# genomicepidemiology/ccphylo

Hardware: AMD Instinct MI355X
Metric: taxa-pairs/sec (dist) + NJ iterations/sec at N taxa, 1/2/4/8 MI355X (higher is better)
Workload: dtype u2 packed codes -> MX-fp4 MFMA (exact integer counts), f64 LT and tree

## Files before the change

### ccphylo_amd/csrc/ccg_dnj_form.h

```cpp
#pragma once
#include <stdlib.h>

#ifdef __HIPCC__
#define CCG_FORM_HD __host__ __device__ __forceinline__
#else
#define CCG_FORM_HD inline
#endif

#define DNJ_B 128
#define DNJ_BANDS 64
#define DNJ_BANDS_MAX 128
#define SEG 2048
#define TBF 1024
#define FIND_RPT 16
#define PLAN_MAXB 256
#define UHIST 64

CCG_FORM_HD int dnj_umax(int n, int seg) { return n > 2 ? (n - 2) / seg + 1 : 1; }

struct DnjGrid {
	int scan_div = 4, scan_max = 2048, seg_mul = 0, prefold_n = 0;
	int small_wave = 0, adapt_rows = 500;
	int sphase_b = 512;
	int plan_help = 256;
	int scan_cmp = 1, cmp_blocks = 1024;
	long long prune_cells = 20000000;
	int prune_on = 1;
	int s_top = 0, s_bands = -1, s_split_n = 16384, plan_qdelay = 2, scan_wave = -1, plan_multi = 1;
	int plan_regsel = 0, plan_fr = FIND_RPT;
	int test_withhold = 0;
	int join_pf = 1;
	int scan_fold = 0;
	int scan_prune = 2;
	int lb = 1, lb_min_n = 16384;
	int lb_groups = 0;
	int scan_vblk = 1;
	void load() {
		if(const char *e = getenv("CCG_JOIN_PF")) join_pf = atoi(e);
		if(const char *e = getenv("CCG_SCAN_FOLD")) scan_fold = atoi(e);
		if(const char *e = getenv("CCG_SCAN_PRUNE")) scan_prune = atoi(e);
		if(const char *e = getenv("CCG_SCAN_VBLK")) scan_vblk = atoi(e);
		if(const char *e = getenv("CCG_S_TOP")) s_top = atoi(e) > 0 ? atoi(e) : 0;
		if(const char *e = getenv("CCG_S_BANDS")) s_bands = atoi(e) >= 0 ? atoi(e) : -1;
		if(const char *e = getenv("CCG_S_SPLIT_N")) s_split_n = atoi(e);
		if(const char *e = getenv("CCG_SCAN_DIV")) scan_div = atoi(e) > 0 ? atoi(e) : 4;
		if(const char *e = getenv("CCG_SCAN_MAX")) scan_max = atoi(e) > 0 ? atoi(e) : 2048;
		if(const char *e = getenv("CCG_SEG_MUL")) seg_mul = atoi(e) > 0 ? atoi(e) : 0;
		if(const char *e = getenv("CCG_PREFOLD_N")) prefold_n = atoi(e) >= 0 ? atoi(e) : 0;
		if(const char *e = getenv("CCG_SCAN_ADAPT")) adapt_rows = atoi(e) > 0 ? atoi(e) : 0;
		if(const char *e = getenv("CCG_SPHASE_BLOCKS")) sphase_b = atoi(e) > 0 ? atoi(e) : 512;
		if(const char *e = getenv("CCG_PLAN_HELP")) plan_help = atoi(e) >= 0 && atoi(e) < 512 ? atoi(e) : 256;
		if(const char *e = getenv("CCG_SCAN_CMP")) scan_cmp = atoi(e);
		if(const char *e = getenv("CCG_PRUNE_CELLS")) prune_cells = atoll(e) > 0 ? atoll(e) : 0;
		prune_on = 1;
		if(const char *e = getenv("CCG_SCAN_CMPB")) cmp_blocks = atoi(e) > 0 ? atoi(e) : 1024;
		if(const char *e = getenv("CCG_PLAN_QDELAY")) plan_qdelay = atoi(e) >= 0 ? atoi(e) : 2;
		if(const char *e = getenv("CCG_SCAN_WAVE")) scan_wave = atoi(e);
		if(const char *e = getenv("CCG_PLAN_MULTI")) plan_multi = atoi(e);
		if(const char *e = getenv("CCG_PLAN_REGSEL")) plan_regsel = atoi(e);
		if(const char *e = getenv("CCG_PLAN_FR")) plan_fr = atoi(e) < 1 ? 1 : atoi(e) > FIND_RPT ? FIND_RPT : atoi(e);
		if(const char *e = getenv("CCG_TEST_WITHHOLD")) test_withhold = atoi(e) & 3;
		if(const char *e = getenv("CCG_SCAN_LB")) lb = atoi(e);
		if(const char *e = getenv("CCG_LB_MIN_N")) lb_min_n = atoi(e);
		if(const char *e = getenv("CCG_LB_GROUPS")) lb_groups = atoi(e);
	}
	int plan_flags(bool prune = false, int helpers = 0) const {
		return (plan_qdelay & 0x3fff) | (test_withhold & 3) << 14 | (plan_regsel ? 0 : 1 << 16) | ((plan_fr - 1) & 15) << 17 | (prune ? 1 << 21 : 0) |
		       (helpers & 511) << 22;
	}
	unsigned plan_blocks(int n) const {
		if(!plan_multi) return 1;
		const int step = (TBF - 64) * plan_fr;
		const int g = (n - 1 + step - 1) / step;
		return (unsigned) (g < 1 ? 1 : g > PLAN_MAXB ? PLAN_MAXB : g);
	}
	int scan_mode(int n, int et = 8) const {
		return scan_wave >= 0 ? scan_wave : n > 16384 || small_wave ? (et == 8 ? 9 : 20) : 0;
	}
	int seg(int n) const {
		int m = seg_mul ? seg_mul : n / (8 * SEG);
		m = m < 1 ? 1 : m > 8 ? 8 : m;
		return m * SEG;
	}
	bool prefold(int n) const { return n > prefold_n; }
	int top(int n) const {
		const int t = s_top ? s_top : n > s_split_n ? 16 : DNJ_B;
		return t < 1 ? 1 : t > DNJ_B ? DNJ_B : t;
	}
	int bands(int n) const {
		int b = s_bands >= 0 ? s_bands : n > s_split_n ? DNJ_BANDS : 0;
		b = b > DNJ_BANDS_MAX ? DNJ_BANDS_MAX : b;
		return top(n) + b > DNJ_B ? DNJ_B - top(n) : b;
	}
	unsigned sphase_blocks() const { return sphase_b; }
	unsigned scan(int n) const {
		const long long g = (n + scan_div - 1) / scan_div;
		return (unsigned) (g < scan_max ? g : scan_max);
	}
};

enum ScanKernel {
	SCAN_BLOCK,
	SCAN_WAVE,
	SCAN_WAVE16,
	SCAN_GROUP,
	SCAN_GROUP_CMP
};
enum ScanSphase {
	SPHASE_NONE,
	SPHASE_SCAN,
	SPHASE_COMPACT
};
struct ScanForm {
	ScanKernel kernel;
	bool stream;
	int G, UC;
	int prune;
	bool cmp;
	bool lb;
	bool tfold;
	int helpers;
	ScanSphase sphase;
	bool fold;
	int sfold;
	unsigned grid;
	int launches;
};

inline int dnj_scan_base(int sm) {
	return sm <= 0 ? 0 : sm < 4 ? 1 : sm == 9 || sm == 21 || sm > 23 ? sm : sm < 20 ? 4 : 20;
}

inline ScanForm dnj_scan_form(const DnjGrid &g, int n, int et, bool gen, bool have_lbm) {
	const int sm = dnj_scan_base(g.scan_mode(n, et));
	const bool grp = sm == 20 || sm == 21, prefold = g.prefold(n);
	const bool fits = dnj_umax(n, g.seg(n)) < UHIST;
	ScanForm f = {};
	f.tfold = prefold && g.scan_fold && sm >= 1;
	if(!gen && g.bands(n) && prefold && sm >= 4 && sm <= 23) {
		if(g.scan_prune == 1 && g.scan_fold) f.prune = 1;
		else if(g.scan_prune == 2 && g.prune_on && !g.scan_fold && (!grp || (g.scan_cmp && fits))) f.prune = 2;
	}
	f.helpers = f.prune == 2 ? g.plan_help : 0;
	f.sphase = f.prune != 2 ? SPHASE_NONE : g.plan_help ? SPHASE_COMPACT : SPHASE_SCAN;
	f.cmp = !gen && sm >= 4 && g.scan_cmp && !f.tfold && f.prune != 1 && fits;
	if(gen || sm < 4) f.kernel = sm >= 1 ? SCAN_WAVE : SCAN_BLOCK;
	else if(have_lbm && f.cmp && grp && g.lb_groups && f.prune == 0) {
		f.kernel = SCAN_GROUP_CMP;
		f.lb = true;
		f.G = 4;
		f.UC = 8;
	} else if(have_lbm && f.cmp) {
		f.kernel = SCAN_WAVE16;
		f.lb = true;
	} else if(grp) {
		f.kernel = f.cmp ? SCAN_GROUP_CMP : SCAN_GROUP;
		f.G = sm == 21 ? 8 : 4;
		f.UC = sm == 21 ? 4 : 8;
	} else {
		f.kernel = SCAN_WAVE16;
		f.stream = sm == 9;
	}
	f.grid = f.cmp && g.scan(n) > (unsigned) g.cmp_blocks ? (unsigned) g.cmp_blocks : g.scan(n);
	f.fold = prefold && !f.tfold;
	f.sfold = f.prune == 2;
	f.launches = 1 + (f.sphase != SPHASE_NONE) + f.fold;
	return f;
// ... 13 lines not shown
```

### ccphylo_amd/csrc/ccg_dnj_search.h

```cpp
#pragma once
#include <stdlib.h>
#include "ccg_tree_common.h"
#include "ccg_dnj_form.h"

struct DenseRows {
	__host__ __device__ __forceinline__ bool owns(long long) const { return true; }
	__host__ __device__ __forceinline__ long long row(long long r) const { return tri(r); }
};

#define SEG_S 1024
#define SEL_RPL 8
#define SEL_STEPS 8
#define FIND_CHUNKS 2048
#define REPLAY_CAP 2048
#define JOIN_UPRE 2048
#define FOLD_BLOCKS 256
#define SRDY_REP 64


template <int ET, bool GEN, int NT, int UNR, class Rows>
__device__ __forceinline__ void row_segment_min(const Rows &rows, const typename Elem<ET>::T *__restrict__ D, double bs,
                                                const double *__restrict__ sD, const int *__restrict__ N, int r,
                                                int c0, int c1, int Nr, double sDr, int isub, int Nm, double sDm,
                                                double &q, int &idx) {
// ... 696 lines not shown
	}
	TSW(1, 10, 64);
	__syncthreads();
	TS(1, 1);
	if(s_done) return;
	auto count_prefix = [&]() {
		constexpr int NC = FR * LW, PER = (NC + 63) / 64;
		int c[PER], sum = 0;
#pragma unroll
		for(int k = 0; k < PER; ++k) {
			const int x = lane * PER + k;
			c[k] = x < NC ? s_mw[x] : 0;
			sum += c[k];
		}
		int tot;
		int pre = wave_excl_scan(sum, &tot);
#pragma unroll
		for(int k = 0; k < PER; ++k) {
			const int x = lane * PER + k;
			if(x < NC) s_mw[x] = pre;
			pre += c[k];
		}
		if(lane == 0) s_cnt = tot;
		return tot;
	};
	if(regsel) {
		const int jsub = s_jsub, isub = s_isub;
		const double m0 = s_m0;
		unsigned long long bs_[FR];
#pragma unroll
		for(int m = 0; m < FR; ++m) {
			bs_[m] = 0ull;
			if(wid > 0) {
				const int r = top - (m * LT + lt);
				qv[m] = r == jsub ? s_Qj : r == isub ? s_Qi : qv[m];
				bs_[m] = __ballot(r >= 1 && qv[m] < m0);
				if(lane == 0) s_mw[m * LW + wid - 1] = __popcll(bs_[m]);
			}
		}
		__syncthreads();
		if(wid == 0) count_prefix();
		__syncthreads();
		const int tot = s_cnt, nt = tot < ktop ? tot : ktop;
		long long ctop = 0;
#pragma unroll
		for(int m = 0; m < FR; ++m) {
			if(bs_[m] == 0ull) continue;
			const int r = top - (m * LT + lt);
			const int pos = s_mw[m * LW + wid - 1] + (int) __builtin_amdgcn_mbcnt_hi(
			                    (unsigned) (bs_[m] >> 32), __builtin_amdgcn_mbcnt_lo((unsigned) bs_[m], 0));
			if(((bs_[m] >> lane) & 1ull) && pos < ktop) {
				sS[pos] = r;
				sQS[pos] = qv[m];
				b.crow[pos] = r;
				b.cbnd[pos] = qv[m];
				if(bid == 0) atomicAdd(&s_uh[dcdiv(r, seg) < UHIST ? dcdiv(r, seg) : UHIST - 1], 1);
				ctop += rows.owns(r) ? r : 0;
			}
		}
		ctop = wave_sum_int(ctop);
		if(lane == 0 && ctop) {
			atomicAdd((unsigned long long *) &ctl->cells, (unsigned long long) ctop);
			atomicAdd((unsigned long long *) &ctl->cells_top, (unsigned long long) ctop);
		}
		__syncthreads();
		if(tid == 0) {
			const int sm = nt == ktop ? sS[ktop - 1] : 1;
			s_nS = s_ntop = nt;
			s_smin = sm;
			ctl->smin = sm;
		}
		__syncthreads();
	}
	const int nS = s_nS, ntop = s_ntop, smin = s_smin, isub = s_isub, jsub = s_jsub;
	const double m0 = s_m0;
	if(wid > 0) {
		double qp = DBL_MAX;
		if(have_rt && rt != isub && rt != jsub && 0 <= dpr) {
			const bool pm = pr == isub;
			qp = qcrit(GEN ? nr : n, GEN ? (pm ? s_Nm : np) : n, dpr, sdr, pm ? s_sDm : sdp);
		}
		spq[lt] = qp;
	}
	TSW(1, 11, 64);
	__syncthreads();
	double U;
	{
		double v = DBL_MAX;
		if(tid < nS) {
			const int r = sS[tid];
			const double qk = tid >= ntop ? sQP[tid] : top - r < NSP ? spq[top - r] : DBL_MAX;
			const double Qk = sQS[tid];
			v = qk > Qk ? qk : Qk;
		}
		const double x = wave_incl_min(v);
		if(wid < 2 && lane == 63) spm[DNJ_B + wid] = x;
		__syncthreads();
		double c = m0;
		if(wid == 1) c = spm[DNJ_B] < c ? spm[DNJ_B] : c;
		if(tid < nS) spm[tid] = x < c ? x : c;
		__syncthreads();
		U = ntop ? spm[ntop - 1] : m0;
	}
	TS(1, 2);
	const bool bands = BANDS && nS > ntop;
	const int nch0 = smin > 1 && bands ? ((smin - 1) >> 6) + 1 : 0;
	const bool table = nch0 <= FIND_CHUNKS;
	const int nch = table ? nch0 : 0;
	for(int c = tid; c < nch; c += TBF) {
		int lo = ntop, hi = nS;
		while(lo < hi) {
			const int mid = (lo + hi) >> 1;
			if(sS[mid] >= 64 * (c + 1)) lo = mid + 1; else hi = mid;
		}
		sch[c] = lo;
	}
	if(nch) __syncthreads();
	auto s_above = [&](int r) {
		int k;
		if(table) {
			k = sch[r >> 6];
			while(k < nS && sS[k] > r) ++k;
		} else {
			int lo = ntop, hi = nS;
			while(lo < hi) {
				const int mid = (lo + hi) >> 1;
				if(sS[mid] > r) lo = mid + 1; else hi = mid;
			}
			k = lo;
		}
		return k;
	};
	int T = ntop, listed = 0;
	long long mycells = 0;
	if(smin > 1 && top - bstep >= 1) {
		double qn[FR];
		for(int base = top - bstep; base >= 1; base -= stride) {
			if(base != top - bstep && wid > 0) {
#pragma unroll
				for(int m = 0; m < FR; ++m) qv[m] = qn[m];
			}
			if(bands) {
				if(tid < FR * LW) {
					const int w = tid / FR, m = tid - (tid / FR) * FR;
					const int rh0 = base - (m * LT + w * 64), rhi = rh0 < smin - 1 ? rh0 : smin - 1;
					const int t0 = rhi >= 1 ? s_above(rhi) : nS;
					s_sb[tid] = t0 ? spm[t0 - 1] : m0;
					s_sf[tid] = t0 < nS && sS[t0] >= rh0 - 63;
				}
				__syncthreads();
			}
			unsigned sfm = 0;
			if(bands && wid > 0) {
				const uint4 f4 = *(const uint4 *) (s_sf + (wid - 1) * FR);
				const unsigned fw[4] = {f4.x, f4.y, f4.z, f4.w};
#pragma unroll
				for(int m = 0; m < FR; ++m) sfm |= ((fw[m >> 2] >> (8 * (m & 3))) & 1u) << m;
			}
			if(base == top) TS(1, 5);
			unsigned long long bm[FR];
			unsigned sbm = 0;
#pragma unroll
			for(int m = 0; m < FR; ++m) bm[m] = 0ull;
			const int mlim = (base - 1) / LT + 1 < fr ? (base - 1) / LT + 1 : fr;
#pragma unroll
			for(int m = 0; m < FR; ++m) {
				if(m >= mlim) continue;
				const int r = wid > 0 ? base - (m * LT + lt) : 0;
				const int rhi = base - (m * LT + (wid - 1) * 64);
				if((jsub <= rhi && jsub >= rhi - 63) || (isub <= rhi && isub >= rhi - 63))
					qv[m] = r == jsub ? s_Qj : r == isub ? s_Qi : qv[m];
				double bnd = U;
				bool srow = false;
				if(bands && wid > 0) {
					if((sfm >> m) & 1u) {
						const int t = s_above(r);
						srow = t < nS && sS[t] == r;
						bnd = t ? spm[t - 1] : m0;
					} else {
						bnd = s_sb[(wid - 1) * FR + m];
					}
				}
				bool f = false;
				if(r >= 1 && r < smin && rows.owns(r)) f = srow || qv[m] < bnd;
				sbm |= (f && srow ? 1u : 0u) << m;
				bm[m] = __ballot(f);
				if(lane == 0 && wid > 0) s_mw[m * LW + wid - 1] = __popcll(bm[m]);
			}
			if(lane == 0 && wid > 0) {
#pragma unroll
				for(int m = 0; m < FR; ++m)
					if(m >= mlim) s_mw[m * LW + wid - 1] = 0;
			}
			if(wid > 0 && base - stride >= 1) {
#pragma unroll
				for(int m = 0; m < FR; ++m) {
					const int r = base - stride - (m * LT + lt);
					qn[m] = m < fr && r >= 1 ? b.Q[r] : DBL_MAX;
				}
			}
			TSW(1, 12, 64);
			if(base == top) TSW(1, 6, 64);
			__syncthreads();
			if(wid == 0) {
				const int tot = count_prefix();
				if(nblk > 1) {
					if(lane == 0 && !(wh_cnt && bid == 0))
						__hip_atomic_store(b.ppub + bid, ((unsigned long long) n << 32) | (unsigned) tot,
						                   __ATOMIC_RELAXED, __HIP_MEMORY_SCOPE_AGENT);
					int off = 0;
					bool stuck = false;
					for(int g0 = 0; g0 < bid; g0 += 64) {
						const int g = g0 + lane;
						unsigned long long u = 0;
						bool ok = g >= bid;
						for(int spin = 0;; ++spin) {
							if(!ok) {
								u = __hip_atomic_load(b.ppub + g, __ATOMIC_RELAXED, __HIP_MEMORY_SCOPE_AGENT);
								ok = (int) (u >> 32) == n;
							}
							if(__all(ok)) break;
							if(spin > spin_max) {
								stuck = true;
								break;
							}
							__builtin_amdgcn_s_sleep(1);
						}
						off += wave_sum_int(g < bid && ok ? (int) (u & 0xffffffffu) : 0);
					}
					if(lane == 0) {
						s_off = off;
						if(stuck) {
							ctl->final_n = -1;
							ctl->done = 1;
						}
					}
				}
				TS(1, 13);
				if(base == top) TS(1, 7);
			}
			__syncthreads();
			if(nblk > 1 && base == top - bstep) T += s_off;
#pragma unroll
			for(int m = 0; m < FR; ++m) {
				if(bm[m] == 0ull) continue;
				const int r = base - (m * LT + lt);
				const bool f = (bm[m] >> lane) & 1ull;
				mycells += f ? r : 0;
				{
					const int rh = base - (m * LT + (wid - 1) * 64), bh0 = dcdiv(rh, seg);
					const int bh = bh0 < UHIST ? bh0 : UHIST - 1;
					const int ch = __popcll(__ballot(f && dcdiv(r, seg) == bh0)), ct = __popcll(bm[m]);
					if(lane == 0) {
						atomicAdd(&s_uh[bh], ch);
						if(ct > ch) atomicAdd(&s_uh[bh0 - 1 < UHIST ? bh0 - 1 : UHIST - 1], ct - ch);
					}
				}
				if(f) {
					const int pos = T + s_mw[m * LW + wid - 1] +
					                (int) __builtin_amdgcn_mbcnt_hi((unsigned) (bm[m] >> 32),
					                                                __builtin_amdgcn_mbcnt_lo((unsigned) bm[m], 0));
					b.crow[pos] = r;
					b.cbnd[pos] = qv[m];
					if(prune) {
						const bool isS = (sbm >> m) & 1u;
						b.eS[pos] = isS;
						if(isS) b.pS_ent[s_above(r)] = pos;
					}
				}
			}
			T += s_cnt;
			listed += s_cnt;
			if(base == top) TSW(1, 8, 64);
			if(base - stride < 1) break;
			__syncthreads();
		}
	}
	TS(1, 3);
	mycells = wave_sum_int(mycells);
	if(lane == 0 && mycells) {
		atomicAdd((unsigned long long *) &ctl->cells, (unsigned long long) mycells);
		atomicAdd((unsigned long long *) &ctl->cells_rest, (unsigned long long) mycells);
	}
	__syncthreads();
	if(tid < UHIST) b.uhist[bid * UHIST + tid] = s_uh[tid];
	if(tid == 0) {
		if(bid == 0) ctl->pblk = nblk;
		if(bid == nblk - 1) ctl->T = T;
		atomicAdd((unsigned long long *) &ctl->rows, (unsigned long long) (listed + (bid == 0 ? ntop : 0)));
	}
	TS(1, 4);
	TS_EXIT(1);
}


struct NoTail {
	__device__ __forceinline__ void begin(const TreeBufs &, int) const {}
	__device__ __forceinline__ void unit(const TreeBufs &b, int, int u, int, int, int, double q, int j) const {
		b.cq[u] = q;
		b.cj[u] = j;
	}
};
struct FoldTail {
	__device__ __forceinline__ void begin(const TreeBufs &, int) const {}
};

template <class Tail>
__device__ __forceinline__ void tail_unit(const Tail &t, const TreeBufs &b, int n, int u, int ua, int ub, int r,
// ... 1249 lines not shown
```

### ccphylo_amd/csrc/ccg_tree_common.h

```cpp
#pragma once
#include <string.h>
#include "ccg_internal.h"

#define TB 256
#define NJ_RB 8
#define NJ_SEG (TB * 8)

struct Entry {
	double f, bnd;
	int row, j;
};

struct TreeCtl {
	int done;
	int final_n;
	int njoins;
	int i, j;
	double Li, Lj, Dij;
	int cand;
	double cand_q;
	int cand_p;
	int pos_i, pos_j;
	int nS, smin;
	int ntop;
// ... 718 lines not shown
#pragma unroll
	for(int e = 0; e < XW_EL; ++e) {
		bad |= !(x[e] >= 0.0 && x[e] <= DBL_MAX);
		if(k0 + e < XS_HEAD) x[e] = 0.0;
	}
	double P = 0, SH = 0;
	int eH = 0;
	if(blk == 0) {
		if(lane == 0) {
			double S = 0;
#pragma unroll
			for(int l = 0; l < XS_HEAD; l += 2) {
				const double2 v = *(const double2 *) (s_row + l);
				S += v.x;
				S += v.y;
			}
			SH = S;
		}
		SH = readlane_d(SH, 0);
		eH = xs_bexp(SH);
		P = SH;
	} else {
		for(int g0 = 0; g0 < blk; g0 += 64) {
			const int g = g0 + lane;
			unsigned long long u = 0;
			bool ok = g >= blk;
			for(int spin = 0;; ++spin) {
				if(!ok) {
					u = __hip_atomic_load(b.xagg + g, __ATOMIC_RELAXED, __HIP_MEMORY_SCOPE_AGENT);
					ok = (unsigned) (u & ((1u << XS_TAG_BITS) - 1)) == tag;
				}
				if(__all(ok)) break;
				if(spin > (1 << 22)) {
					stuck = true;
					break;
				}
				__builtin_amdgcn_s_sleep(2);
			}
			const double a = g < blk && ok ? __longlong_as_double((long long) (u & ~((1ull << XS_TAG_BITS) - 1))) : 0.0;
			P += wave_sum_fixed(a);
		}
	}
	int ep_c = xs_bexp(P);
	const int ex0 = ep_c;
	bad |= P != 0.0 && ep_c == 0;
	int nc = 0, nt = 0;
	double acc = 0;
	{
		const double cs = x[0] + x[1] + x[2] + x[3];
		double xs = cs;
#define S_(C, R_) xs += dpp_d<C, R_>(0.0, xs);
		CCG_DPP_STEPS(S_)
#undef S_
		double Pl = P + (xs - cs);
		double Pn[XW_EL];
		int en[XW_EL];
#pragma unroll
		for(int e = 0; e < XW_EL; ++e) {
			Pl += x[e];
			Pn[e] = Pl;
			en[e] = xs_bexp(Pl);
		}
		const int epl = dpp_i<DPP_WAVE_SHR1, 0xF>(ep_c, en[XW_EL - 1]);
		unsigned cm = 0, tm = 0;
		double fl[XW_EL], run = 0;
#pragma unroll
		for(int e = 0; e < XW_EL; ++e) {
			const int ep = e ? en[e - 1] : epl;
			const double t = ldexp(x[e], 1075 - ep) + 0.5;
			fl[e] = floor(t);
			cm |= (unsigned) (ep != en[e]) << e;
			tm |= (unsigned) (t == fl[e]) << e;
			run += fl[e];
		}
		tm &= ~cm;
		ep_c = __builtin_amdgcn_readlane(en[XW_EL - 1], 63);
		const unsigned long long fm = __ballot((cm | tm) != 0u);
		if(fm == 0ull) {
			acc = wave_sum_fixed(run);
		} else {
			XsCross *xc = b.xcr + (size_t) blk * XB_CAP;
			XsTie *xt = b.xti + (size_t) blk * XB_CAP_T;
			int from = 0;
			bool tied = false;
			double acc_t = 0;
			for(unsigned long long f = fm; f; f &= f - 1) {
				const int L = __ffsll((long long) f) - 1;
				acc += wave_sum_fixed(lane >= from && lane < L ? run : 0.0);
				const unsigned cmL = __builtin_amdgcn_readlane(cm, L), tmL = __builtin_amdgcn_readlane(tm, L);
#pragma unroll
				for(int e = 0; e < XW_EL; ++e) {
					const double fe = readlane_d(fl[e], L);
					const int k = TB * blk + XW_EL * L + e;
					if((cmL >> e) & 1u) {
						if(nc < XB_CAP && lane == 0) {
							XsCross r;
							r.v = readlane_d(x[e], L);
							r.run = acc;
							r.k = k;
							r.x = __builtin_amdgcn_readlane(en[e], L);
							r.R = 0;
							r.tb = nt;
							xc[nc] = r;
						}
						++nc;
						acc = 0;
						tied = false;
					} else if((tmL >> e) & 1u) {
						if(!tied) {
							if(nt < XB_CAP_T && lane == 0) {
								XsTie r;
								r.k = k;
								r.pi = (xs_par(acc) + xs_par(fe) + 1) & 1;
								r.R = nc;
								r.first = nc == 0;
								xt[nt] = r;
							}
							++nt;
							tied = true;
							acc += fe;
						} else {
							const bool up = xs_par(acc - acc_t + (fe - 1.0)) != 0;
							acc += up ? fe : fe - 1.0;
						}
						acc_t = acc;
					} else {
						acc += fe;
					}
				}
				from = L + 1;
			}
			acc += wave_sum_fixed(lane >= from ? run : 0.0);
		}
	}
	bad |= ep_c == 0x7FF;
	const int why = (__any(bad) ? XS_WHY_VALUE : 0) | (__any(stuck) ? XS_WHY_STUCK : 0) |
	                (nc > XB_CAP ? XS_WHY_NC : 0) | (nt > XB_CAP_T ? XS_WHY_NT : 0);
	if(lane == 0) {
		XsBlk s;
		s.tail = acc;
		s.head = SH;
		s.nc = nc;
		s.nt = nt;
		s.tp = xs_par(acc);
		s.ex0 = ex0;
		s.eh = eH;
		s.bad = why;
		s.pad0 = s.pad1 = 0;
		b.xblk[blk] = s;
	}
	(void) n;
}

#define XS_PRE_C 2
#define XS_PRE_H 4
struct XsPre {
	XsBlk blk, bh[XS_PRE_H - 1];
	XsCross cr[XS_PRE_C];
	XsTie ti;
};
__device__ __forceinline__ void xs_prefetch(const TreeBufs &b, int G, XsPre &p) {
	const int g = threadIdx.x & 63;
	if(g < G) {
		p.blk = b.xblk[g];
#pragma unroll
		for(int c = 0; c < XS_PRE_C; ++c) p.cr[c] = b.xcr[(size_t) g * XB_CAP + c];
		p.ti = b.xti[(size_t) g * XB_CAP_T];
	}
#pragma unroll
	for(int h = 1; h < XS_PRE_H; ++h)
		if(g + 64 * h < G) p.bh[h - 1] = b.xblk[g + 64 * h];
}

__device__ bool xs_walk_blocks(const TreeBufs &b, int G, double *out, const XsPre *pre, int n, int *why_out) {
	(void) n;
	__shared__ XsCross lc[XS_CAP];
	__shared__ int lcR[XS_CAP], lcT[XS_CAP];
	__shared__ XsTie lt[XS_CAP_T];
	__shared__ int ltR[XS_CAP_T];
	__shared__ double lseg[XS_CAP + 1];
	const int lane = threadIdx.x & 63;
	for(int q = lane; q <= XS_CAP; q += 64) lseg[q] = 0.0;
	const double SH = b.xblk[0].head;
	const int eH = b.xblk[0].eh;
	int cob = 0, tob = 0, Rwb = 0;
	int why = 0;
	wave_sync();
	const bool allpre = pre && G <= 64 * XS_PRE_H && b.xs_allpre;
	__shared__ int bco[64 * XS_PRE_H], bto[64 * XS_PRE_H], bRw[64 * XS_PRE_H], bex[64 * XS_PRE_H];
	__shared__ short cown[XS_CAP], town[XS_CAP_T];
	for(int g0 = 0; g0 < G; g0 += 64) {
		const int g = g0 + lane, ph = g0 >> 6;
		XsBlk s;
		if(g < G) {
			s = pre && g0 == 0 ? pre->blk
			    : allpre       ? pre->bh[ph >= 1 && ph < XS_PRE_H ? ph - 1 : 0]
			                   : b.xblk[g];
		} else {
			s.tail = 0;
			s.nc = s.nt = s.tp = s.ex0 = s.bad = 0;
		}
		why |= s.bad | (s.nc > XB_CAP ? XS_WHY_NC : 0) | (s.nt > XB_CAP_T ? XS_WHY_NT : 0);
		int tc, tt, tr;
		const int co = cob + wave_excl_scan(s.nc, &tc);
		const int to = tob + wave_excl_scan(s.nt, &tt);
		const int Rw = Rwb + wave_excl_scan(s.tp, &tr);
		if(allpre) {
			bco[g0 + lane] = co;
			bto[g0 + lane] = to;
			bRw[g0 + lane] = Rw;
			bex[g0 + lane] = s.ex0;
			if(g < G) {
				for(int c = 0; c < s.nc && c < XB_CAP && co + c < XS_CAP; ++c) cown[co + c] = (short) g;
				for(int t = 0; t < s.nt && t < XB_CAP_T && to + t < XS_CAP_T; ++t) town[to + t] = (short) g;
			}
		} else {
			for(int c = 0; c < s.nc && c < XB_CAP; ++c) {
				if(co + c < XS_CAP) {
					lc[co + c] = pre && g0 == 0 && c < XS_PRE_C ? pre->cr[c < XS_PRE_C ? c : 0] : b.xcr[(size_t) g * XB_CAP + c];
					lcR[co + c] = Rw;
					lcT[co + c] = to;
				}
			}
			for(int t = 0; t < s.nt && t < XB_CAP_T; ++t) {
				if(to + t < XS_CAP_T) {
					lt[to + t] = pre && g0 == 0 && t == 0 ? pre->ti : b.xti[(size_t) g * XB_CAP_T + t];
					ltR[to + t] = Rw;
				}
			}
		}
		wave_sync();
		if(g < G) {
			if(!allpre) {
				const int want = co == 0 ? eH : co - 1 < XS_CAP ? lc[co - 1].x : -1;
				why |= s.ex0 != want ? XS_WHY_EX0 : 0;
			}
			if(co + s.nc <= XS_CAP) atomicAdd(&lseg[co + s.nc], s.tail);
			else why |= XS_WHY_CAP;
		}
		cob += tc;
		tob += tt;
		Rwb += tr;
	}
	const int nx = cob, ntot = tob;
	if(allpre) {
		auto owner = [&](const short *own, int q) { return (int) own[q]; };
		XsCross cv[2];
		int cg[2];
#pragma unroll
		for(int m = 0; m < 2; ++m) {
			const int q = lane + 64 * m;
			cg[m] = -1;
			if(q < nx && q < XS_CAP) {
				const int g = owner(cown, q);
				cg[m] = g;
				cv[m] = b.xcr[(size_t) g * XB_CAP + (q - bco[g])];
			}
		}
		XsTie tv[XS_CAP_T / 64];
		int tg[XS_CAP_T / 64];
#pragma unroll
		for(int m = 0; m < XS_CAP_T / 64; ++m) {
			const int q = lane + 64 * m;
			tg[m] = -1;
			if(q < ntot && q < XS_CAP_T) {
				const int g = owner(town, q);
				tg[m] = g;
				tv[m] = b.xti[(size_t) g * XB_CAP_T + (q - bto[g])];
			}
		}
#pragma unroll
		for(int m = 0; m < 2; ++m) {
			const int q = lane + 64 * m;
			if(cg[m] >= 0) {
				lc[q] = cv[m];
				lcR[q] = bRw[cg[m]];
				lcT[q] = bto[cg[m]];
			}
		}
#pragma unroll
		for(int m = 0; m < XS_CAP_T / 64; ++m) {
			const int q = lane + 64 * m;
			if(tg[m] >= 0) {
				lt[q] = tv[m];
				ltR[q] = bRw[tg[m]];
			}
		}
		wave_sync();
		for(int g = lane; g < G; g += 64) {
			const int co = bco[g];
			const int want = co == 0 ? eH : co - 1 < XS_CAP ? lc[co - 1].x : -1;
			why |= bex[g] != want ? XS_WHY_EX0 : 0;
		}
	}
	why |= nx > XS_CAP - 1 || ntot > XS_CAP_T ? XS_WHY_CAP : 0;
#pragma unroll
	for(int q = 0; q < XS_NWHY; ++q) why |= __any((why >> q) & 1) ? 1 << q : 0;
	*why_out = why;
	if(why) return false;
	wave_sync();
	TS(4, 7);
	double A0[2], A1[2], cvA[2];
	int exA[2], cxA[2];
#pragma unroll
	for(int h = 0; h < 2; ++h) {
		const int s = lane + 64 * h;
		A0[h] = A1[h] = cvA[h] = 0.0;
		exA[h] = cxA[h] = 0;
		if(s <= nx) {
			double seg = lseg[s];
			int ta = 0, tz = ntot, Rc = 0;
			if(s) {
				const XsCross &p = lc[s - 1];
				exA[h] = p.x;
				ta = lcT[s - 1] + p.tb;
				Rc = lcR[s - 1];
			} else {
				exA[h] = eH;
			}
			if(s < nx) {
				const XsCross &q = lc[s];
				cvA[h] = q.v;
				cxA[h] = q.x;
				seg += q.run;
				tz = lcT[s] + q.tb;
			}
			int dn0 = 0, dn1 = 0;
			for(int g = ta; g < tz; ++g) {
				const XsTie &t = lt[g];
				int pi = t.pi;
				if(t.first) pi ^= (ltR[g] - Rc) & 1;
				dn0 += 1 - ((pi + dn0) & 1);
				dn1 += 1 - ((1 + pi + dn1) & 1);
			}
			A0[h] = seg - (double) dn0;
			A1[h] = seg - (double) dn1;
		}
	}
	TS(4, 8);
	double S = SH;
	bool ok = (eH > 0 && eH < 0x7FF) || (SH == 0.0 && lseg[0] == 0.0);
	for(int s = 0; s <= nx; ++s) {
		const int h = s >> 6, l = s & 63;
		if(s > 0 || eH > 0) {
			const int exs = __builtin_amdgcn_readlane(h ? exA[1] : exA[0], l);
			const double a0 = readlane_d(h ? A0[1] : A0[0], l), a1 = readlane_d(h ? A1[1] : A1[0], l);
			const int ue = exs - 1075;
			ok = ok && exs > 0 && exs < 0x7FF && xs_bexp(S) == exs;
			const double T0 = ldexp(S, -ue);
			const double T = T0 + (((unsigned) __double_as_longlong(T0) & 1u) ? a1 : a0);
			ok = ok && T < 9007199254740992.0;
			S = ldexp(T, ue);
		}
		if(s < nx) {
			const double Sn = S + readlane_d(h ? cvA[1] : cvA[0], l);
			ok = ok && xs_bexp(Sn) == __builtin_amdgcn_readlane(h ? cxA[1] : cxA[0], l);
			S = Sn;
		}
	}
	TS(4, 9);
#if defined(CCG_TRACE) && !defined(CCG_DNJ_NO_TRACE)
	if(blockIdx.x == 0 && threadIdx.x == 0) {
		const int s_ = g_trace_hi - n;
		if(s_ >= 0 && s_ < 256) {
			const unsigned long long t0 = ~g_trace[(s_ * NKT + 4) * 16 + 15];
			g_trace[(s_ * NKT + 4) * 16 + 10] = t0 + (unsigned long long) nx * 100;
			g_trace[(s_ * NKT + 4) * 16 + 11] = t0 + (unsigned long long) ntot * 100;
		}
	}
#endif
	*out = S;
	if(!ok) *why_out = XS_WHY_WALK;
	return ok;
}

__device__ void row_sum_j_wave(const TreeBufs &b, int n, bool exact, bool general, double *sd, int *nj, bool *need,
                               bool *chain) {
	const int G = (int) cdiv(n, TB);
	XsPre pre;
	if(exact) xs_prefetch(b, G, pre);
	TS(4, 5);
	fold_update_wave(b, G, exact, general, sd, nj, need);
	TS(4, 6);
	*chain = false;
	if(*need) {
		double r;
		int why = 0;
		if(xs_walk_blocks(b, G, &r, exact ? &pre : nullptr, n, &why)) {
			*sd = r;
		} else {
			*chain = true;
			if(blockIdx.x == 0 && (threadIdx.x & 63) == 0)
				for(int q = 0; q < XS_NWHY; ++q)
					if((why >> q) & 1) atomicAdd(&b.ctl->xs_why[q], 1);
		}
	}
}

#define XS_NT 512
#define XS_RB 6
template <int UNUSED = 0>
__global__ __launch_bounds__(XS_NT) void k_exact_sum(TreeBufs b, int n, int G) {
	__shared__ double s_sd;
	__shared__ int s_nj, s_need, s_stop;
	TreeCtl *ctl = b.ctl;
	if(threadIdx.x < 64) {
		const int done = ctl->done;
		double sd = 0;
		int nj = 0;
		bool need = false;
		if(!done) fold_update_wave(b, G, true, false, &sd, &nj, &need);
		if(threadIdx.x == 0) {
			s_stop = done;
			s_sd = sd;
			s_nj = nj;
			s_need = need;
		}
	}
	__syncthreads();
	if(s_stop) return;
	double r = s_sd;
	bool chain = false;
	if(s_need && !exact_sum_w<XS_NT, XS_RB>(b.contrib, n, &r)) {
		r = serial_sum_t<XS_NT>(b.contrib, n);
		chain = true;
	}
	if(threadIdx.x == 0) {
		ctl->xsum = r;
		ctl->xnj = s_nj;
		ctl->serial_sums += s_need;
		ctl->chain_sums += chain;
	}
}

__device__ __forceinline__ void qk_take(double &bq, int &bk, double q, int k) {
	if(q < bq || (q == bq && k > bk)) {
		bq = q;
		bk = k;
	}
}

template <int NT>
__device__ __forceinline__ void qk_block_reduce(double &bq, int &bk, double *sq, int *sk) {
	for(int o = 32; o > 0; o >>= 1) {
		const double oq = __shfl_xor(bq, o, 64);
		const int ok = __shfl_xor(bk, o, 64);
		qk_take(bq, bk, oq, ok);
	}
	const int lane = threadIdx.x & 63, wid = threadIdx.x >> 6;
	if(lane == 0) {
		sq[wid] = bq;
		sk[wid] = bk;
	}
	__syncthreads();
	if(threadIdx.x == 0) {
		for(int w = 1; w < NT / 64; ++w) qk_take(bq, bk, sq[w], sk[w]);
	}
}

__device__ __forceinline__ void qk_fold_wave(const double *pq, const int *pk, int G, double &bq, int &bk) {
	const int lane = threadIdx.x & 63;
	bq = DBL_MAX;
	bk = -1;
	for(int g = lane; g < G; g += 64) qk_take(bq, bk, pq[g], pk[g]);
	for(int o = 32; o > 0; o >>= 1) {
		const double oq = __shfl_xor(bq, o, 64);
		const int ok = __shfl_xor(bk, o, 64);
		qk_take(bq, bk, oq, ok);
	}
}

__device__ __forceinline__ void qf_wave_reduce(double &q, long long &f) {
#define S_(C, R)                                          \
	{                                                     \
		const double oq_ = dpp_d<C, R>(DBL_MAX, q);       \
		const long long of_ = dpp_l<C, R>(-2, f);         \
		if(oq_ < q || (oq_ == q && of_ > f)) {            \
			q = oq_;                                      \
			f = of_;                                      \
		}                                                 \
	}
	CCG_DPP_STEPS(S_)
#undef S_
	q = readlane_d(q, 63);
	f = readlane_l(f, 63);
}


struct KTimer {
	bool on;
	hipStream_t st;
	hipEvent_t ev[1025];
	int cls[1025];
	int used;
	long long cnt[CCG_NKSTAT], ns[CCG_NKSTAT];
	void init(hipStream_t s, bool enable) {
		if(on)
			for(int k = 0; k < 1025; ++k) hipEventDestroy(ev[k]);
		on = enable;
		st = s;
		used = 0;
		memset(cnt, 0, sizeof(cnt));
		memset(ns, 0, sizeof(ns));
		if(on) {
			for(int k = 0; k < 1025; ++k) hipEventCreate(&ev[k]);
			hipEventRecord(ev[0], st);
			used = 1;
		}
	}
	void harvest() {
		hipEventSynchronize(ev[used - 1]);
		for(int k = 1; k < used; ++k) {
			float ms = 0;
			hipEventElapsedTime(&ms, ev[k - 1], ev[k]);
			cnt[cls[k]] += 1;
			ns[cls[k]] += (long long) (ms * 1.0e6);
		}
		hipEvent_t t = ev[0];
		ev[0] = ev[used - 1];
		ev[used - 1] = t;
		used = 1;
	}
	void mark(int c) {
		if(!on) return;
		cls[used] = c;
		hipEventRecord(ev[used++], st);
		if(used == 1025) harvest();
	}
	void finish() {
		if(!on) return;
		harvest();
		for(int k = 0; k < 1025; ++k) hipEventDestroy(ev[k]);
		on = false;
	}
};
```

### ccphylo_amd/csrc/tree.hip

```cpp
#include <string.h>
#include <stdio.h>
#include <vector>
#include <stdlib.h>
#include "ccg_tree_common.h"

#include "ccg_dnj_search.h"

static thread_local DnjGrid g_grid;

template <int ET>
__global__ __launch_bounds__(TB) void k_init_rows(const typename Elem<ET>::T *__restrict__ D, int n, double bs,
                                                  double *__restrict__ sD, int *__restrict__ N, TreeCtl *ctl) {
	__shared__ double buf[TB / 64][64];
	const int lane = threadIdx.x & 63, wid = threadIdx.x >> 6;
	const int k = blockIdx.x * (TB / 64) + wid;
	if(k >= n) return;
	double s = 0;
	int c = 1, miss = 0;
	const typename Elem<ET>::T *row = D + tri(k);
	for(int m0 = 0; m0 < k; m0 += 64) {
		int m = m0 + lane;
		double d = m < k ? Elem<ET>::get(row[m], bs) : 0.0;
		bool ok = m < k && 0 <= d;
		miss |= m < k && !ok;
// ... 1618 lines not shown
			else launch_scan_v<ET, false>(f, st, D, bs, b, n, seg);
			break;
		case SCAN_GROUP:
		case SCAN_GROUP_CMP:
			if(f.lb) k_dnj_scan_gc<ET, 4, 8, false, true><<<f.grid, TB, 0, st>>>(D, bs, b, n, seg);
			else if(f.G == 8) launch_scan_g<ET, 8, 4>(f, st, D, bs, b, n, seg);
			else launch_scan_g<ET, 4, 8>(f, st, D, bs, b, n, seg);
			break;
	}
}

template <int ET, bool GEN>
static int enqueue_iteration(hipStream_t st, typename Elem<ET>::T *D, double bs, const TreeBufs &b, int n, int first,
                             int method, int exact, KTimer &kt) {
	const unsigned gn = cdiv(n, TB);
	const int general = GEN;
	const int xs = 0;
	if(method == CCG_TREE_DNJ) {
		const int seg = g_grid.seg(n), prefold = g_grid.prefold(n);
		const ScanForm f = dnj_scan_form(g_grid, n, ET, GEN, b.lbm != NULL);
		enqueue_plan<ET, GEN>(st, D, bs, b, n, first, f);
		kt.mark(CCG_K_FIND);
		if(f.sphase == SPHASE_COMPACT) k_dnj_sphase<ET, false><<<g_grid.sphase_blocks(), TB, 0, st>>>(D, bs, b, n, seg);
		else if(f.sphase == SPHASE_SCAN) k_dnj_sphase<ET><<<g_grid.sphase_blocks(), TB, 0, st>>>(D, bs, b, n, seg);
		enqueue_scan<ET, GEN>(f, st, D, bs, b, n, seg);
		if(f.fold) k_dnj_fold<><<<FOLD_BLOCKS, TB, 0, st>>>(b, n, seg, f.sfold);
		kt.mark(CCG_K_REST);
		if(prefold && g_grid.join_pf) k_dnj_join_pf<ET, GEN><<<gn, TB, 0, st>>>(D, bs, b, n, general, g_grid.join_pf == 2);
		else k_dnj_join<ET, GEN><<<gn, TB, 0, st>>>(D, bs, b, n, general, prefold, seg);
		if(GEN) k_update_general<ET><<<1, 1024, 0, st>>>(D, bs, b, n);
		kt.mark(CCG_K_UPDATE);
		if(xs) {
			k_exact_sum<><<<1, XS_NT, 0, st>>>(b, n, (int) gn);
			kt.mark(CCG_K_XSUM);
		}
		if(g_grid.bands(n - 1) && g_grid.scan_vblk && dnj_scan_form(g_grid, n - 1, ET, GEN, b.lbm != NULL).prune)
			k_dnj_requeue<ET, true, true><<<gn, TB, 0, st>>>(D, bs, b, n, general, exact);
		else if(g_grid.bands(n - 1)) k_dnj_requeue<ET, true><<<gn, TB, 0, st>>>(D, bs, b, n, general, exact);
		else k_dnj_requeue<ET, false><<<gn, TB, 0, st>>>(D, bs, b, n, general, exact);
		kt.mark(CCG_K_REQUEUE);
		return (GEN ? 4 : 3) + f.launches + xs;
	}
	if(method == CCG_TREE_HNJ) {
		k_hnj_argmin<><<<gn, TB, 0, st>>>(b, n);
		kt.mark(CCG_K_ARGMIN);
		k_nj_join<ET><<<gn, TB, 0, st>>>(D, bs, b, n, (int) gn, general, DBL_MAX);
		if(GEN) k_update_general<ET><<<1, 1024, 0, st>>>(D, bs, b, n);
		kt.mark(CCG_K_UPDATE);
		if(xs) {
			k_exact_sum<><<<1, XS_NT, 0, st>>>(b, n, (int) gn);
			kt.mark(CCG_K_XSUM);
		}
		k_hnj_update<ET><<<gn, TB, 0, st>>>(D, bs, b, n, general, exact);
		kt.mark(CCG_K_POP);
		return (GEN ? 4 : 3) + xs;
	}
	const unsigned g = (unsigned) nj_blocks(n);
	if(method == CCG_TREE_MN) k_nj_argmin<ET, GEN, true><<<g, TB, 0, st>>>(D, bs, b, n);
	else k_nj_argmin<ET, GEN><<<g, TB, 0, st>>>(D, bs, b, n);
	kt.mark(CCG_K_ARGMIN);
	k_nj_join<ET><<<gn, TB, 0, st>>>(D, bs, b, n, (int) g, general, method == CCG_TREE_MN ? DBL_MAX : 1.0);
	if(GEN) k_update_general<ET><<<1, 1024, 0, st>>>(D, bs, b, n);
	kt.mark(CCG_K_UPDATE);
	if(xs) {
		k_exact_sum<><<<1, XS_NT, 0, st>>>(b, n, (int) gn);
		kt.mark(CCG_K_XSUM);
	}
	k_nj_pop<ET><<<gn, TB, 0, st>>>(D, b, n, general, exact);
	kt.mark(CCG_K_POP);
	return (GEN ? 4 : 3) + xs;
}

static bool g_progress = false;

template <int ET>
static int tree_run_t(ccg_ctx *ctx, const ccg_tree_args *a, void *Dd, ccg_join *joins, int *njoins,
                      int *final_n, double *final_d, int64_t *stats, const ccg_dnj_state *sin,
                      ccg_dnj_state *sout) {
	typedef typename Elem<ET>::T T;
	T *D = (T *) Dd;
	const int n0 = a->n;
	const double bs = a->byteScale;
	hipStream_t st = ctx->stream;
	TreeWork w;
	g_grid = DnjGrid();
	g_grid.load();
	g_progress = getenv("CCG_PROGRESS") != nullptr;
	const bool cmp_env = getenv("CCG_SCAN_CMPB") != nullptr;
	auto cmp_share = [&](int blocks) {
		return ctx->cus > 0 && ctx->cus < ctx->ncu ? (blocks * ctx->cus / ctx->ncu > 64 ? blocks * ctx->cus / ctx->ncu : 64)
		                                           : blocks;
	};
	if(!cmp_env) g_grid.cmp_blocks = cmp_share(g_grid.cmp_blocks);
	int rc = tree_alloc_ctx(ctx, &w, n0);
	if(rc) return rc;
	TreeBufs b = w.b;
	TreeCtl init;
	memset(&init, 0, sizeof(init));
	init.neg = (a->flags & 2) != 0;
	init.exact = a->exact != 0;
	init.method = a->method;
	init.hj = init.hi = -1;
	if(sin) {
		init.cand = sin->cand;
		init.cand_q = sin->Q[sin->cand];
		init.cand_p = sin->P[sin->cand];
	}
	CCG_CHECK(hipMemcpyAsync(b.ctl, &init, sizeof(init), hipMemcpyHostToDevice, st));
	long long launches = 0;
	static thread_local KTimer kt;
	CCG_CHECK(hipEventRecord(ctx->ev0, st));
	kt.init(st, a->profile != 0);
	k_init_rows<ET><<<cdiv(n0, TB / 64), TB, 0, st>>>(D, n0, bs, b.sD, b.N, b.ctl);
	k_init_cols<ET><<<cdiv(n0, TB), TB, 0, st>>>(D, n0, bs, b.sD, b.N, b.ctl);
	launches += 2;
	bool resumed_counts = false;
	if(sin) {
		CCG_CHECK(hipMemcpyAsync(b.sD, sin->sD, (size_t) n0 * 8, hipMemcpyHostToDevice, st));
		CCG_CHECK(hipMemcpyAsync(b.Q, sin->Q, (size_t) n0 * 8, hipMemcpyHostToDevice, st));
		CCG_CHECK(hipMemcpyAsync(b.N, sin->N, (size_t) n0 * 4, hipMemcpyHostToDevice, st));
		CCG_CHECK(hipMemcpyAsync(b.P, sin->P, (size_t) n0 * 4, hipMemcpyHostToDevice, st));
		for(int k = 0; k < n0 && !resumed_counts; ++k) resumed_counts = sin->N[k] != n0;
	} else if(a->method == CCG_TREE_DNJ) {
		k_init_hnj<ET><<<cdiv(n0, TB / 64), TB, 0, st>>>(DenseRows(), D, n0, bs, b.sD, b.N, b.Q, b.P);
		k_dnj_prep<><<<1, TB, 0, st>>>(b, n0);
		launches += 2;
	} else if(a->method == CCG_TREE_HNJ) {
		k_init_hnj<ET><<<cdiv(n0, TB / 64), TB, 0, st>>>(DenseRows(), D, n0, bs, b.sD, b.N, b.Q, b.P);
		launches += 1;
	}
	kt.mark(CCG_K_INIT);
	CCG_CHECK(hipGetLastError());
	TreeCtl h;
	CCG_CHECK(hipMemcpyAsync(&h, b.ctl, sizeof(h), hipMemcpyDeviceToHost, st));
	CCG_CHECK(hipStreamSynchronize(st));
	const bool general = h.has_missing != 0 || resumed_counts;
	void *lbmem = NULL;
	if(a->method == CCG_TREE_DNJ && !general && g_grid.lb && n0 > g_grid.lb_min_n) {
		const long long LS = (n0 + LBW - 1) / LBW;
		const size_t lbb = ((size_t) n0 * LS * 4 + 255) & ~(size_t) 255;
		const size_t msb = ((size_t) (LS + 1) * 8 + 255) & ~(size_t) 255;
		const size_t ubb = ((size_t) n0 * 8 + 255) & ~(size_t) 255, skb = (size_t) (LB_SCAN + LB_HELP) * LB_SLOT * 8;
		if(ccg_ctx_workspace(ctx, 1, lbb + msb + ubb + skb, &lbmem) == CCG_OK) {
			b.lbm = (unsigned *) lbmem;
			b.msd = (double *) ((char *) lbmem + lbb);
			b.ubq = (double *) ((char *) lbmem + lbb + msb);
			b.lbs = LS;
			b.lbskip = (long long *) ((char *) lbmem + lbb + msb + ubb);
			CCG_CHECK(hipMemsetAsync(b.lbskip, 0, skb, st));
			k_lb_init<ET><<<cdiv(n0, TB / 64), TB, 0, st>>>(D, n0, bs, b);
			launches += 1;
			CCG_CHECK(hipGetLastError());
			if(!getenv("CCG_SCAN_PRUNE")) g_grid.scan_prune = 0;
			if(!cmp_env) g_grid.cmp_blocks = cmp_share(2048);
		} else {
			(void) hipGetLastError();
			lbmem = NULL;
		}
	}
#ifdef CCG_TRACE
	const char *tn = getenv("CCG_TRACE_N");
	int trace_hi = tn ? atoi(tn) : n0 / 2;
	CCG_CHECK(hipMemcpyToSymbolAsync(HIP_SYMBOL(g_trace_hi), &trace_hi, sizeof(int), 0, hipMemcpyHostToDevice, st));
	static unsigned long long zero_tr[256 * 4 * 16];
	CCG_CHECK(hipMemcpyToSymbolAsync(HIP_SYMBOL(g_trace), zero_tr, sizeof(zero_tr), 0, hipMemcpyHostToDevice, st));
#endif
	int n = n0;
	int since_check = 0;
	long long win_rows = h.rows, win_cells = h.cells;
	bool stopped = false;
	const int stop_n = a->max_joins > 0 && a->max_joins < n0 - 2 ? n0 - a->max_joins : 2;
	while(n > stop_n) {
		launches += general ? enqueue_iteration<ET, true>(st, D, bs, b, n, n == n0, a->method, a->exact, kt)
		                    : enqueue_iteration<ET, false>(st, D, bs, b, n, n == n0, a->method, a->exact, kt);
		CCG_CHECK(hipGetLastError());
		--n;
		if(++since_check == 1024) {
			since_check = 0;
			CCG_CHECK(hipMemcpyAsync(&h, b.ctl, sizeof(h), hipMemcpyDeviceToHost, st));
			CCG_CHECK(hipStreamSynchronize(st));
			g_grid.small_wave = g_grid.adapt_rows && h.rows - win_rows > 1024LL * g_grid.adapt_rows;
			g_grid.prune_on = !g_grid.prune_cells || h.cells - win_cells > 1024LL * g_grid.prune_cells;
			win_rows = h.rows;
			win_cells = h.cells;
			if(g_progress && (n0 - n) % (16 * 1024) == 0)
				fprintf(stderr, "ccg_tree: %d joins, n = %d, rows %lld cells %lld (reference rule %lld / %lld)\n", n0 - n,
				        n, h.rows, h.cells, h.ref_rows, h.ref_cells);
			if(h.done) {
				stopped = true;
				break;
			}
		}
	}
	(void) stopped;
	CCG_CHECK(hipEventRecord(ctx->ev1, st));
	kt.finish();
	CCG_CHECK(hipMemcpyAsync(&h, b.ctl, sizeof(h), hipMemcpyDeviceToHost, st));
	CCG_CHECK(hipStreamSynchronize(st));
	if(b.lbskip) {
		std::vector<long long> sl((size_t) (LB_SCAN + LB_HELP) * LB_SLOT);
		CCG_CHECK(hipMemcpyAsync(sl.data(), b.lbskip, sl.size() * 8, hipMemcpyDeviceToHost, st));
		CCG_CHECK(hipStreamSynchronize(st));
		for(size_t x = 0; x < (size_t) LB_SCAN + LB_HELP; ++x) {
			h.cells_lbskip += sl[x * LB_SLOT];
			h.cells_help -= sl[x * LB_SLOT + 1];
		}
	}
	float ms = 0;
	CCG_CHECK(hipEventElapsedTime(&ms, ctx->ev0, ctx->ev1));
	if(getenv("CCG_XS_WHY"))
		fprintf(stderr, "xs_why: value %d nc %d nt %d stuck %d ex0 %d cap %d walk %d (chain sums %d of %d)\n",
		        h.xs_why[0], h.xs_why[1], h.xs_why[2], h.xs_why[3], h.xs_why[4], h.xs_why[5], h.xs_why[6],
		        h.chain_sums, h.serial_sums);
#ifdef CCG_TRACE
	{
		static unsigned long long tr[256 * NKT * 16];
		CCG_CHECK(hipMemcpyFromSymbol(tr, HIP_SYMBOL(g_trace), sizeof(tr), 0, hipMemcpyDeviceToHost));
		const int nk = a->method == CCG_TREE_DNJ ? NKT : 0;
		double acc[NKT][16] = {{0}}, gap[NKT] = {0}, itv = 0;
		int cnt = 0;
		bool present[NKT] = {false};
		for(int s = 0; s < 256; ++s)
			for(int k = 0; k < nk; ++k) present[k] = present[k] || tr[(s * NKT + k) * 16 + 15];
		for(int s = 0; s < 256; ++s) {
			const unsigned long long *e = tr + s * NKT * 16;
			bool ok = true;
			for(int k = 0; k < nk; ++k) ok = ok && (!present[k] || (e[k * 16 + 15] && e[k * 16 + 14]));
			if(!ok) continue;
			++cnt;
			int k0 = 0, prev = -1;
			while(k0 < nk && !present[k0]) ++k0;
			for(int k = k0; k < nk; ++k) {
				if(!present[k]) continue;
				unsigned long long t0 = ~e[k * 16 + 15];
				for(int p = 0; p < 15; ++p)
					if(e[k * 16 + p]) acc[k][p] += ((double) e[k * 16 + p] - (double) t0) / 100.0;
				if(prev >= 0) gap[k] += ((double) t0 - (double) e[prev * 16 + 14]) / 100.0;
				prev = k;
			}
			if(s + 1 < 256 && tr[((s + 1) * NKT + k0) * 16 + 15]) {
				gap[k0] += ((double) ~tr[((s + 1) * NKT + k0) * 16 + 15] - (double) e[(nk - 1) * 16 + 14]) / 100.0;
				itv += ((double) ~tr[((s + 1) * NKT + k0) * 16 + 15] - (double) ~e[k0 * 16 + 15]) / 100.0;
			}
		}
		const char *kn[NKT] = {"select", "plan/find", "scan", "join", "requeue"};
		fprintf(stderr, "trace: %d joins at n <= %d; iteration %.2f us; serial replays %d, serial sums %d\n", cnt,
		        trace_hi, cnt ? itv / (cnt - 1) : 0, h.serial_replays, h.serial_sums);
		{
			static unsigned long long sp[256 * 64 * 3];
			CCG_CHECK(hipMemcpyFromSymbol(sp, HIP_SYMBOL(g_samp), sizeof(sp), 0, hipMemcpyDeviceToHost));
			double st_max = 0, en_max = 0, dur = 0, st_med = 0, stg = 0;
			int sc = 0, jc = 0;
			for(int s = 0; s < 256; ++s) {
				const unsigned long long t0 = ~tr[(s * NKT + 2) * 16 + 15];
				if(!tr[(s * NKT + 2) * 16 + 15]) continue;
				double smax = 0, emax = 0;
				int any = 0;
				for(int q = 0; q < 64; ++q) {
					const unsigned long long *e = sp + (s * 64 + q) * 3;
					if(!e[0] || !e[2] || e[0] < t0) continue;
					const double a = (e[0] - t0) / 100.0, z = (e[2] - t0) / 100.0;
					smax = a > smax ? a : smax;
					emax = z > emax ? z : emax;
					dur += z - a;
					if(e[1] >= e[0]) stg += (e[1] - e[0]) / 100.0;
					st_med += a;
					++sc;
					any = 1;
				}
				if(any) {
					st_max += smax;
					en_max += emax;
					++jc;
				}
			}
			{
				static unsigned long long ua[256 * 64 * 8];
				CCG_CHECK(hipMemcpyFromSymbol(ua, HIP_SYMBOL(g_uamp), sizeof(ua), 0, hipMemcpyDeviceToHost));
				double ud[4] = {0}, ug[4] = {0}, us0 = 0;
				int uc[4] = {0}, gc[4] = {0}, s0c = 0;
				for(int s = 0; s < 256; ++s) {
					const unsigned long long t0 = ~tr[(s * NKT + 2) * 16 + 15];
					if(!tr[(s * NKT + 2) * 16 + 15]) continue;
					for(int q = 0; q < 64; ++q) {
						const unsigned long long *e = ua + (s * 64 + q) * 8;
						const unsigned long long *sp0 = sp + (s * 64 + q) * 3;
						if(e[0] && e[0] >= t0 && sp0[0] && e[0] >= sp0[0]) {
							us0 += (e[0] - sp0[0]) / 100.0;
							++s0c;
						}
						for(int k = 0; k < 4; ++k) {
							if(e[2 * k] && e[2 * k + 1] >= e[2 * k] && e[2 * k] >= t0) {
								ud[k] += (e[2 * k + 1] - e[2 * k]) / 100.0;
								++uc[k];
							}
							if(k && e[2 * k] && e[2 * k - 1] && e[2 * k] >= e[2 * k - 1] && e[2 * k] >= t0) {
								ug[k] += (e[2 * k] - e[2 * k - 1]) / 100.0;
								++gc[k];
							}
						}
					}
				}
				fprintf(stderr, "  scan units (wave 0 of sampled blocks): entry->first unit %.2f us;", s0c ? us0 / s0c : 0.0);
				for(int k = 0; k < 4; ++k)
					fprintf(stderr, " unit%d n=%d dur %.2f gap %.2f;", k, uc[k], uc[k] ? ud[k] / uc[k] : 0.0, gc[k] ? ug[k] / gc[k] : 0.0);
				fprintf(stderr, "\n");
				memset(ua, 0, sizeof(ua));
// ... 149 lines not shown
```

Measured before the change: 198.9 million.

## Size compaction scan grid from occupancy, halve find repeat, inline exact-sum walk

```diff
diff --git a/ccphylo_amd/csrc/ccg_dnj_form.h b/ccphylo_amd/csrc/ccg_dnj_form.h
--- a/ccphylo_amd/csrc/ccg_dnj_form.h
+++ b/ccphylo_amd/csrc/ccg_dnj_form.h
@@ -12,7 +12,7 @@
 #define DNJ_BANDS_MAX 128
 #define SEG 2048
 #define TBF 1024
-#define FIND_RPT 16
+#define FIND_RPT 8
 #define PLAN_MAXB 256
 #define UHIST 64
 
diff --git a/ccphylo_amd/csrc/ccg_dnj_search.h b/ccphylo_amd/csrc/ccg_dnj_search.h
--- a/ccphylo_amd/csrc/ccg_dnj_search.h
+++ b/ccphylo_amd/csrc/ccg_dnj_search.h
@@ -872,8 +872,10 @@
 			}
 			unsigned sfm = 0;
 			if(bands && wid > 0) {
-				const uint4 f4 = *(const uint4 *) (s_sf + (wid - 1) * FR);
-				const unsigned fw[4] = {f4.x, f4.y, f4.z, f4.w};
+				static_assert(FR % 4 == 0, "a wave's FR flag bytes are read as whole words");
+				unsigned fw[FR / 4];
+#pragma unroll
+				for(int w = 0; w < FR / 4; ++w) fw[w] = ((const unsigned *) (s_sf + (wid - 1) * FR))[w];
 #pragma unroll
 				for(int m = 0; m < FR; ++m) sfm |= ((fw[m >> 2] >> (8 * (m & 3))) & 1u) << m;
 			}
diff --git a/ccphylo_amd/csrc/ccg_tree_common.h b/ccphylo_amd/csrc/ccg_tree_common.h
--- a/ccphylo_amd/csrc/ccg_tree_common.h
+++ b/ccphylo_amd/csrc/ccg_tree_common.h
@@ -894,6 +894,33 @@
 	(void) n;
 }
 
+__device__ __forceinline__ void xs_copy(XsBlk &d, const XsBlk &s) {
+	d.tail = s.tail;
+	d.head = s.head;
+	d.nc = s.nc;
+	d.nt = s.nt;
+	d.tp = s.tp;
+	d.ex0 = s.ex0;
+	d.eh = s.eh;
+	d.bad = s.bad;
+	d.pad0 = s.pad0;
+	d.pad1 = s.pad1;
+}
+__device__ __forceinline__ void xs_copy(XsCross &d, const XsCross &s) {
+	d.v = s.v;
+	d.run = s.run;
+	d.k = s.k;
+	d.x = s.x;
+	d.R = s.R;
+	d.tb = s.tb;
+}
+__device__ __forceinline__ void xs_copy(XsTie &d, const XsTie &s) {
+	d.k = s.k;
+	d.pi = s.pi;
+	d.R = s.R;
+	d.first = s.first;
+}
+
 #define XS_PRE_C 2
 #define XS_PRE_H 4
 struct XsPre {
@@ -904,17 +931,20 @@
 __device__ __forceinline__ void xs_prefetch(const TreeBufs &b, int G, XsPre &p) {
 	const int g = threadIdx.x & 63;
 	if(g < G) {
-		p.blk = b.xblk[g];
-#pragma unroll
-		for(int c = 0; c < XS_PRE_C; ++c) p.cr[c] = b.xcr[(size_t) g * XB_CAP + c];
-		p.ti = b.xti[(size_t) g * XB_CAP_T];
-	}
-#pragma unroll
-	for(int h = 1; h < XS_PRE_H; ++h)
-		if(g + 64 * h < G) p.bh[h - 1] = b.xblk[g + 64 * h];
-}
-
-__device__ bool xs_walk_blocks(const TreeBufs &b, int G, double *out, const XsPre *pre, int n, int *why_out) {
+		xs_copy(p.blk, b.xblk[g]);
+#pragma unroll
+		for(int c = 0; c < XS_PRE_C; ++c) xs_copy(p.cr[c], b.xcr[(size_t) g * XB_CAP + c]);
+		xs_copy(p.ti, b.xti[(size_t) g * XB_CAP_T]);
+	}
+	if(b.xs_allpre) {
+		if(g + 64 < G) xs_copy(p.bh[0], b.xblk[g + 64]);
+		if(g + 128 < G) xs_copy(p.bh[1], b.xblk[g + 128]);
+		if(g + 192 < G) xs_copy(p.bh[2], b.xblk[g + 192]);
+	}
+}
+
+__device__ __forceinline__ bool xs_walk_blocks(const TreeBufs &b, int G, double *out, const XsPre &pre, bool have_pre, int n,
+                                               int *why_out) {
 	(void) n;
 	__shared__ XsCross lc[XS_CAP];
 	__shared__ int lcR[XS_CAP], lcT[XS_CAP];
@@ -928,16 +958,23 @@
 	int cob = 0, tob = 0, Rwb = 0;
 	int why = 0;
 	wave_sync();
-	const bool allpre = pre && G <= 64 * XS_PRE_H && b.xs_allpre;
+	const bool allpre = have_pre && G <= 64 * XS_PRE_H && b.xs_allpre;
 	__shared__ int bco[64 * XS_PRE_H], bto[64 * XS_PRE_H], bRw[64 * XS_PRE_H], bex[64 * XS_PRE_H];
 	__shared__ short cown[XS_CAP], town[XS_CAP_T];
 	for(int g0 = 0; g0 < G; g0 += 64) {
 		const int g = g0 + lane, ph = g0 >> 6;
 		XsBlk s;
 		if(g < G) {
-			s = pre && g0 == 0 ? pre->blk
-			    : allpre       ? pre->bh[ph >= 1 && ph < XS_PRE_H ? ph - 1 : 0]
-			                   : b.xblk[g];
+			if(have_pre && g0 == 0) {
+				xs_copy(s, pre.blk);
+			} else if(allpre) {
+				static_assert(XS_PRE_H == 4, "bh[] is picked by written-out compares");
+				xs_copy(s, pre.bh[0]);
+				if(ph == 2) xs_copy(s, pre.bh[1]);
+				if(ph == 3) xs_copy(s, pre.bh[2]);
+			} else {
+				xs_copy(s, b.xblk[g]);
+			}
 		} else {
 			s.tail = 0;
 			s.nc = s.nt = s.tp = s.ex0 = s.bad = 0;
@@ -959,14 +996,25 @@
 		} else {
 			for(int c = 0; c < s.nc && c < XB_CAP; ++c) {
 				if(co + c < XS_CAP) {
-					lc[co + c] = pre && g0 == 0 && c < XS_PRE_C ? pre->cr[c < XS_PRE_C ? c : 0] : b.xcr[(size_t) g * XB_CAP + c];
+					static_assert(XS_PRE_C == 2, "the prefetched crossings are picked by a compare");
+					XsCross x;
+					if(have_pre && g0 == 0 && c < XS_PRE_C) {
+						xs_copy(x, pre.cr[0]);
+						if(c) xs_copy(x, pre.cr[1]);
+					} else {
+						xs_copy(x, b.xcr[(size_t) g * XB_CAP + c]);
+					}
+					xs_copy(lc[co + c], x);
 					lcR[co + c] = Rw;
 					lcT[co + c] = to;
 				}
 			}
 			for(int t = 0; t < s.nt && t < XB_CAP_T; ++t) {
 				if(to + t < XS_CAP_T) {
-					lt[to + t] = pre && g0 == 0 && t == 0 ? pre->ti : b.xti[(size_t) g * XB_CAP_T + t];
+					XsTie x;
+					if(have_pre && g0 == 0 && t == 0) xs_copy(x, pre.ti);
+					else xs_copy(x, b.xti[(size_t) g * XB_CAP_T + t]);
+					xs_copy(lt[to + t], x);
 					ltR[to + t] = Rw;
 				}
 			}
@@ -996,7 +1044,7 @@
 			if(q < nx && q < XS_CAP) {
 				const int g = owner(cown, q);
 				cg[m] = g;
-				cv[m] = b.xcr[(size_t) g * XB_CAP + (q - bco[g])];
+				xs_copy(cv[m], b.xcr[(size_t) g * XB_CAP + (q - bco[g])]);
 			}
 		}
 		XsTie tv[XS_CAP_T / 64];
@@ -1008,14 +1056,14 @@
 			if(q < ntot && q < XS_CAP_T) {
 				const int g = owner(town, q);
 				tg[m] = g;
-				tv[m] = b.xti[(size_t) g * XB_CAP_T + (q - bto[g])];
+				xs_copy(tv[m], b.xti[(size_t) g * XB_CAP_T + (q - bto[g])]);
 			}
 		}
 #pragma unroll
 		for(int m = 0; m < 2; ++m) {
 			const int q = lane + 64 * m;
 			if(cg[m] >= 0) {
-				lc[q] = cv[m];
+				xs_copy(lc[q], cv[m]);
 				lcR[q] = bRw[cg[m]];
 				lcT[q] = bto[cg[m]];
 			}
@@ -1024,7 +1072,7 @@
 		for(int m = 0; m < XS_CAP_T / 64; ++m) {
 			const int q = lane + 64 * m;
 			if(tg[m] >= 0) {
-				lt[q] = tv[m];
+				xs_copy(lt[q], tv[m]);
 				ltR[q] = bRw[tg[m]];
 			}
 		}
@@ -1116,7 +1164,7 @@
 	return ok;
 }
 
-__device__ void row_sum_j_wave(const TreeBufs &b, int n, bool exact, bool general, double *sd, int *nj, bool *need,
+__device__ __forceinline__ void row_sum_j_wave(const TreeBufs &b, int n, bool exact, bool general, double *sd, int *nj, bool *need,
                                bool *chain) {
 	const int G = (int) cdiv(n, TB);
 	XsPre pre;
@@ -1128,7 +1176,7 @@
 	if(*need) {
 		double r;
 		int why = 0;
-		if(xs_walk_blocks(b, G, &r, exact ? &pre : nullptr, n, &why)) {
+		if(xs_walk_blocks(b, G, &r, pre, exact, n, &why)) {
 			*sd = r;
 		} else {
 			*chain = true;
diff --git a/ccphylo_amd/csrc/tree.hip b/ccphylo_amd/csrc/tree.hip
--- a/ccphylo_amd/csrc/tree.hip
+++ b/ccphylo_amd/csrc/tree.hip
@@ -1794,7 +1794,22 @@
 			launches += 1;
 			CCG_CHECK(hipGetLastError());
 			if(!getenv("CCG_SCAN_PRUNE")) g_grid.scan_prune = 0;
-			if(!cmp_env) g_grid.cmp_blocks = cmp_share(2048);
+			if(!cmp_env) {
+				int per_cu = 0, pc2 = 0;
+				hipError_t e0 = hipOccupancyMaxActiveBlocksPerMultiprocessor(
+				    &per_cu, (const void *) k_dnj_scan_v<ET, DenseRows, NoTail, false, 0, true, true>, TB, 0);
+				hipError_t e2 = hipOccupancyMaxActiveBlocksPerMultiprocessor(
+				    &pc2, (const void *) k_dnj_scan_v<ET, DenseRows, NoTail, false, 2, true, true>, TB, 0);
+				if(g_grid.scan_prune == 2 && pc2 < per_cu) per_cu = pc2;
+				const int cus = ctx->cus > 0 && ctx->cus < ctx->ncu ? ctx->cus : ctx->ncu;
+				const int round = per_cu * cus;
+				if(e0 != hipSuccess || e2 != hipSuccess || round < 1) {
+					(void) hipGetLastError();
+					g_grid.cmp_blocks = cmp_share(2048);
+				} else {
+					g_grid.cmp_blocks = 2 * round <= g_grid.scan_max || round > g_grid.scan_max ? 2 * round : round;
+				}
+			}
 		} else {
 			(void) hipGetLastError();
 			lbmem = NULL;
```

Result: no change. 200.1 million (median of 6 runs) (+0.6%).
